# SilvioWeging/kASA

Hardware: AMD Instinct MI355X
Metric: reads/s in identify (10M x 150bp vs k=12 index) (higher is better)
Workload: dtype u64

## Files before the change

kasa_amd/csrc/kasa_hip.hip:

```cpp
#include <hip/hip_runtime.h>
#include <chrono>
#include <cstdlib>
#include <cstring>
#include <rocprim/device/device_radix_sort.hpp>
#include <rocprim/device/device_segmented_radix_sort.hpp>
#include <rocprim/iterator/transform_iterator.hpp>
#include <rocprim/device/device_scan.hpp>
#include <rocprim/functional.hpp>
#include <rocprim/iterator/counting_iterator.hpp>

#include <algorithm>
#include <cstdarg>
#include <cstdint>
#include <cstdio>
#include <cstring>
#include <map>
#include <mutex>
#include <new>
#include <string>
#include <thread>
#include <type_traits>
#include <vector>

#include <dlfcn.h>
// ... 4921 lines not shown
#pragma unroll
        for (int c = 0; c < HELD; ++c) if ((uint32_t)c * 64u < m) pass1((uint32_t)c * 64u, held[c]);
        for (uint32_t i0 = HELD * 64u; i0 < m; i0 += 64) {
            const uint32_t i = i0 + lane;
            pass1(i0, i < m ? st[s0 + i] : make_uint2(RK_FINAL, 0u));
        }
        LDS_WAVE_SYNC();
        uint32_t carry = 0;
        for (uint32_t w0 = 0; w0 < W; w0 += 64) {
            const uint32_t w = w0 + lane;
            const uint32_t pc = (w < W) ? (uint32_t)__popc(bm[w]) : 0u;
            uint32_t incl = pc;
            incl = wave_incl_sum(incl);
            if (w < W) pre[w] = carry + incl - pc;
            carry += lane_value<63>(incl);
        }
        const uint32_t nSlots = carry;
        LDS_WAVE_SYNC();
        auto pass2 = [&](uint32_t i0, uint2 e) {
            const uint32_t i = i0 + lane;
            bool pending = false;
            uint32_t slot = 0;
            float sc = 0.0f;
            if (i < m) {
                const uint32_t kind = e.x >> 30;
                if (kind != 2u) {
                    const uint32_t t = e.x & 0xFFFFFu;
                    slot = pre[t >> 5] + (uint32_t)__popc(bm[t >> 5] & ((1u << (t & 31u)) - 1u));
                    slotTax[slot] = t;
                    if (kind == 1u) val[slot] = __uint_as_float(e.y);
                    else { pending = true; if (kind == 0u) sc = event_score(evT, kHigh - (int)rk_level(e.x), e.y >> 16); }
                }
            }
            while (__ballot(pending) != 0ull) {
                if (pending) atomicMin(&claim[slot], (uint32_t)lane);
                LDS_WAVE_SYNC();
                if (pending && claim[slot] == (uint32_t)lane) {
                    float v = val[slot];
                    if ((e.x >> 30) == 3u) {
                        const int kF = (int)((e.x >> 20) & 31u), kL = (int)(e.y & 31u);
                        const int step = (e.x & RK_SEG_DESC) ? -1 : 1;
                        for (int k = step > 0 ? kF : kL, c = kL - kF; c >= 0; --c, k += step)
                            v = __fadd_rn(v, event_score(evT, k, seg_size(e.y, k == kF)));
                    } else
                        for (uint32_t j = 0; j < (e.y & 0xFFFFu); ++j) v = __fadd_rn(v, sc);
                    val[slot] = v;
                    claim[slot] = 0xFFFFFFFFu;
                    pending = false;
                }
                LDS_WAVE_SYNC();
            }
        };
#pragma unroll
        for (int c = 0; c < HELD; ++c) if ((uint32_t)c * 64u < m) pass2((uint32_t)c * 64u, held[c]);
        for (uint32_t i0 = HELD * 64u; i0 < m; i0 += 64) {
            const uint32_t i = i0 + lane;
            pass2(i0, i < m ? st[s0 + i] : make_uint2(0u, 0u));
        }
        LDS_WAVE_SYNC();
        for (uint32_t sl = lane; sl < nSlots; sl += 64) st[s0 + sl] = make_uint2(slotTax[sl], __float_as_uint(val[sl]));
        if (lane == 0) rowLen[r] = nSlots;
        LDS_WAVE_SYNC();
#pragma unroll
        for (int c = 0; c < HELD; ++c) held[c] = ahead[c];
    }
}

static constexpr int PR_THREADS = 256, PR_ITEMS = 8;
__global__ __launch_bounds__(PR_THREADS) void profile_reduce_kernel(const uint64_t *__restrict__ sorted, uint32_t nKeys, uint32_t nTaxa,
                                                                     uint64_t *__restrict__ cntUnique, uint64_t *__restrict__ hiTab,
                                                                     uint64_t *__restrict__ midTab, uint64_t *__restrict__ loTab, ProfLayout PL)
{
    __shared__ unsigned long long sSum[PR_THREADS / 64];
    __shared__ uint64_t sEdge[2];
    const uint64_t mask = (1ull << PL.bits()) - 1ull;
    auto add = [&](uint64_t key, uint64_t c) {
        const uint32_t tax = (uint32_t)(key & ((1ull << PL.tb) - 1ull));
        if (c == 0 || tax == (1u << PL.tb) - 1u) return;
        const uint32_t n = (uint32_t)((key >> PL.tb) & ((1ull << PL.nb) - 1ull));
        const uint32_t lv = (uint32_t)(key >> (PL.tb + PL.nb));
        const size_t cell = (size_t)lv * nTaxa + tax;
        if (n == 1) atomicAdd((unsigned long long *)&cntUnique[cell], (unsigned long long)c);
        fixed_add(hiTab, midTab, loTab, cell, c, n);
    };
    const uint32_t chunk = PR_THREADS * PR_ITEMS;
    for (uint64_t base = (uint64_t)blockIdx.x * chunk; base < nKeys; base += (uint64_t)gridDim.x * chunk) {
        const uint64_t i0 = base + threadIdx.x * PR_ITEMS;
        uint64_t v[PR_ITEMS];
        if (i0 + PR_ITEMS <= nKeys) {
#pragma unroll
            for (int j = 0; j < PR_ITEMS; j += 2) {
                const ulonglong2 w = *reinterpret_cast<const ulonglong2 *>(sorted + i0 + j);
                v[j] = w.x; v[j + 1] = w.y;
            }
        } else {
#pragma unroll
            for (int j = 0; j < PR_ITEMS; ++j) v[j] = (i0 + j < nKeys) ? sorted[i0 + j] : ~0ull;
        }
        if (threadIdx.x == 0) sEdge[0] = (v[0] >> 16) & mask;
        const uint32_t lastIdx = (base + chunk <= nKeys) ? chunk - 1 : (uint32_t)(nKeys - 1 - base);
        if (threadIdx.x == lastIdx / PR_ITEMS) sEdge[1] = (v[lastIdx % PR_ITEMS] >> 16) & mask;
        __syncthreads();
        const bool uniform = sEdge[0] == sEdge[1];
        if (uniform) {
            unsigned long long sum = 0;
#pragma unroll
            for (int j = 0; j < PR_ITEMS; ++j) if (i0 + j < nKeys) sum += v[j] & 0xFFFFull;
            for (int off = 32; off > 0; off >>= 1) sum += __shfl_down(sum, off);
            if ((threadIdx.x & 63) == 0) sSum[threadIdx.x >> 6] = sum;
            __syncthreads();
            if (threadIdx.x == 0) {
                unsigned long long total = 0;
                for (int w = 0; w < PR_THREADS / 64; ++w) total += sSum[w];
                add(sEdge[0], total);
            }
        } else {
            uint64_t cur = (v[0] >> 16) & mask, acc = 0;
#pragma unroll
            for (int j = 0; j < PR_ITEMS; ++j) {
                if (i0 + j >= nKeys) break;
                const uint64_t k = (v[j] >> 16) & mask;
                if (k != cur) { add(cur, acc); cur = k; acc = 0; }
                acc += v[j] & 0xFFFFull;
            }
            add(cur, acc);
        }
        __syncthreads();
    }
}

static constexpr int PT_THREADS = 1024, PT_LEFT = 2048;
struct ProfTableLayout { uint8_t nn[MAX_LEVELS]; uint16_t first[MAX_LEVELS + 1]; int lvLo, lvHi; };
static ProfTableLayout prof_table_layout(int nK, int lvLo, int lvHi, uint32_t nTaxa, uint64_t budgetCells)
{
    ProfTableLayout L;
    memset(&L, 0, sizeof(L));
    L.lvLo = lvLo; L.lvHi = lvHi;
    const uint64_t perTaxon = nTaxa ? budgetCells / nTaxa : 0;
    const int nW = lvHi - lvLo;
    if (nW <= 0 || perTaxon < (uint64_t)nW) { L.lvHi = lvLo; return L; }
    uint64_t left = perTaxon - (uint64_t)nW;
    for (int lv = lvLo; lv < lvHi; ++lv) L.nn[lv] = 1;
    auto grow = [&](int lv, uint64_t upTo) { while (lv >= lvLo && lv < lvHi && L.nn[lv] < upTo && left > 0) { ++L.nn[lv]; --left; } };
    for (int lv = lvLo; lv < lvHi; ++lv) grow(lv, 2);
    if (lvHi == nK) {
        grow(nK - 2, 4);
        grow(nK - 1, 24);
        grow(nK - 2, 8);
    }
    for (uint64_t upTo = 3; upTo <= 8; ++upTo) for (int lv = lvHi - 1; lv >= lvLo; --lv) grow(lv, upTo);
    for (int lv = 0; lv < MAX_LEVELS; ++lv) L.first[lv + 1] = (uint16_t)(L.first[lv] + L.nn[lv]);
    return L;
}
__global__ __launch_bounds__(PT_THREADS) void profile_table_kernel(const uint64_t *__restrict__ keys, uint32_t nKeys, uint32_t nTaxa, int nK, ProfTableLayout TL,
                                                                   uint64_t *__restrict__ cntUnique, uint64_t *__restrict__ hiTab,
                                                                   uint64_t *__restrict__ midTab, uint64_t *__restrict__ loTab, ProfLayout PL,
                                                                   uint64_t *__restrict__ leftOut, unsigned long long *__restrict__ leftCursor)
{
    extern __shared__ uint32_t tab[];
    __shared__ uint64_t sLeft[PT_LEFT];
    __shared__ uint32_t sLeftN;
    __shared__ unsigned long long sLeftBase;
    const uint32_t cells = (uint32_t)TL.first[MAX_LEVELS] * nTaxa;
    for (uint32_t i = threadIdx.x; i < cells; i += PT_THREADS) tab[i] = 0u;
    if (threadIdx.x == 0) sLeftN = 0;
    __syncthreads();
    const uint64_t mask = (1ull << PL.bits()) - 1ull;
    auto flush0 = [&]() {
        const uint32_t n = min(sLeftN, (uint32_t)PT_LEFT);
        if (threadIdx.x == 0) sLeftBase = atomicAdd(leftCursor, (unsigned long long)n);
        __syncthreads();
        for (uint32_t i = threadIdx.x; i < n; i += PT_THREADS) leftOut[sLeftBase + i] = sLeft[i];
        __syncthreads();
        if (threadIdx.x == 0) sLeftN = 0;
        __syncthreads();
    };
    constexpr int PT_KEYS = 8;
    const uint64_t step = (uint64_t)gridDim.x * PT_THREADS * PT_KEYS;
    const uint64_t rounds = ((uint64_t)nKeys + step - 1) / step;
    const uint32_t maxHits = (uint32_t)std::min<uint64_t>(65535ull, 0xFFFFFFFFull / std::max<uint64_t>(1, rounds * PT_THREADS * PT_KEYS));
    auto &flush = flush0;
    for (uint64_t rd = 0; rd < rounds; ++rd) {
        const uint64_t i0 = rd * step + (uint64_t)blockIdx.x * PT_THREADS * PT_KEYS + threadIdx.x;
        uint64_t kk[PT_KEYS];
#pragma unroll
        for (int q = 0; q < PT_KEYS; ++q) { const uint64_t i = i0 + (uint64_t)q * PT_THREADS; kk[q] = i < nKeys ? keys[i] : 0ull; }
#pragma unroll
        for (int q = 0; q < PT_KEYS; ++q) {
            const uint64_t key = kk[q];
            const uint64_t f = (key >> 16) & mask;
            const uint32_t hits = (uint32_t)(key & 0xFFFFull);
            const uint32_t tax = (uint32_t)(f & ((1ull << PL.tb) - 1ull));
            if (hits != 0u && tax != (1u << PL.tb) - 1u) {
                const uint32_t n = (uint32_t)((f >> PL.tb) & ((1ull << PL.nb) - 1ull));
                const uint32_t lv = (uint32_t)(f >> (PL.tb + PL.nb));
                if ((int)lv < TL.lvLo || (int)lv >= TL.lvHi) {}
                else if (n >= 1u && n <= (uint32_t)TL.nn[lv] && hits <= maxHits) atomicAdd(&tab[((uint32_t)TL.first[lv] + (n - 1u)) * nTaxa + tax], hits);
                else {
                    const uint32_t at = atomicAdd(&sLeftN, 1u);
                    if (at < (uint32_t)PT_LEFT) sLeft[at] = key;
                    else leftOut[atomicAdd(leftCursor, 1ull)] = key;
                }
            }
        }
        __syncthreads();
        if (sLeftN > (uint32_t)(PT_LEFT / 2)) flush();
    }
    flush();
    for (uint32_t i = threadIdx.x; i < cells; i += PT_THREADS) {
        const uint32_t c = tab[i];
        if (!c) continue;
        const uint32_t tax = i % nTaxa, row = i / nTaxa;
        uint32_t lv = 0;
        while (row >= (uint32_t)TL.first[lv + 1]) ++lv;
        const uint32_t n = row - (uint32_t)TL.first[lv] + 1u;
        const size_t cell = (size_t)lv * nTaxa + tax;
        if (n == 1u) atomicAdd((unsigned long long *)&cntUnique[cell], (unsigned long long)c);
        fixed_add(hiTab, midTab, loTab, cell, c, n);
    }
}

__global__ __launch_bounds__(256) void row_copy_kernel(const uint32_t *__restrict__ rowPos, const uint32_t *__restrict__ rowLen,
                                const uint64_t *__restrict__ rowOff, uint32_t nReads, const uint2 *__restrict__ st,
                                uint32_t *__restrict__ outTax, float *__restrict__ outScore)
{
    const int lane = threadIdx.x & 63, wv = threadIdx.x >> 6;
    const uint32_t waves = gridDim.x * 4u;
    for (uint32_t r = blockIdx.x * 4u + wv; r < nReads; r += waves) {
        const uint32_t s = rowPos[r];
        const uint32_t m = rowLen[r] & ~ROW_MERGE;
        const uint64_t o = rowOff[r];
        for (uint32_t i = lane; i < m; i += 64) { const uint2 e = st[s + i]; outTax[o + i] = e.x; outScore[o + i] = __uint_as_float(e.y); }
    }
}

__global__ void widen_kernel(const uint32_t *__restrict__ in, uint64_t *__restrict__ out, uint32_t n)
{
    const uint32_t i = blockIdx.x * blockDim.x + threadIdx.x;
    if (i < n) out[i] = in[i] & 0x7FFFFFFFu;
}

__global__ void invert_kernel(const uint32_t *__restrict__ plist, uint32_t n, uint32_t *__restrict__ slotOf)
{
    const uint32_t i = blockIdx.x * blockDim.x + threadIdx.x;
    if (i < n) slotOf[plist[i]] = i;
}

static int slots_from_reads(kasa_ctx *c)
{
    const uint64_t nQ = c->nQ;
    int rc;
    if ((rc = c->plist.reserve(nQ * 4 + 64)) || (rc = c->slotBuf.reserve(nQ * 4 + 64)) || (rc = c->qReadA.reserve(nQ * 4 + 64))) return rc;
    hipEvent_t a, b;
    if ((rc = timer_begin(c, c->timers[KASA_STAGE_REGROUP], &a, &b))) return rc;
    if (nQ) {
        unsigned bits = 1;
        while ((1ull << bits) < (uint64_t)std::max<int64_t>(c->nReads, 1)) ++bits;
        rocprim::counting_iterator<uint32_t> iota(0);
        size_t tmpBytes = 0;
        HIPCHK(rocprim::radix_sort_pairs(nullptr, tmpBytes, c->qRead, c->qReadA.as<uint32_t>(), iota, c->plist.as<uint32_t>(),
                                         (size_t)nQ, 0u, bits, c->stream));
        if ((rc = c->sortTmp.reserve(tmpBytes))) return rc;
        HIPCHK(rocprim::radix_sort_pairs(c->sortTmp.p, tmpBytes, c->qRead, c->qReadA.as<uint32_t>(), iota, c->plist.as<uint32_t>(),
                                         (size_t)nQ, 0u, bits, c->stream));
        invert_kernel<<<blocks_for(nQ, 256), 256, 0, c->stream>>>(c->plist.as<uint32_t>(), (uint32_t)nQ, c->slotBuf.as<uint32_t>());
        HIPCHK(hipGetLastError());
    }
    if ((rc = timer_end(c, c->timers[KASA_STAGE_REGROUP], a, b))) return rc;
    c->slotOf = c->slotBuf.as<uint32_t>();
    return KASA_OK;
}

template <int RW>
static int launch_group(kasa_ctx *c, const uint32_t *slotOf, uint32_t nTiles, uint32_t cap, uint32_t keyCap, int cov, unsigned long long *cursor, bool coop,
                        const uint32_t *tileList = nullptr, uint32_t nListed = 0)
{
    const uint64_t nQ = c->nQ;
    uint32_t *needCoop = reinterpret_cast<uint32_t *>(cursor + 3);
    const uint32_t grid = tileList ? nListed : nTiles;
#define KASA_GROUP_ARGS(KEY, META) c->keys<KEY>(), c->depth.as<uint8_t>(), c->rep.as<uint32_t>(), slotOf, (uint32_t)nQ, \
        c->tileNext.as<uint32_t>(), nTiles, c->ix->meta.as<META>(), c->ix->tax.as<uint32_t>(), (uint32_t)c->ix->n, \
        c->kHigh, c->kLow, c->recOut ? c->recOut : c->rec.as<uint32_t>(), c->pool.as<uint32_t>(), cap, cursor, cov, c->cntTotal.as<uint64_t>(), c->ix->nTaxa, \
        c->profKeys.as<uint64_t>(), keyCap, cursor + 2, prof_layout(c->ix->nTaxa, c->nK), c->cntAllHi.as<uint64_t>(), c->cntAllMid.as<uint64_t>(), c->cntAllLo.as<uint64_t>(), needCoop, tileList, c->recOut ? (uint32_t)RW : c->recCW
    if (c->ix->wide && RW == 16 && c->nK == 19)
        group_kernel<RW, key128, RW == 16 ? 19 : 0><<<grid, GTHREADS, 0, c->stream>>>(KASA_GROUP_ARGS(key128, uint16_t));
    else if (c->ix->wide)
        group_kernel<RW, key128, 0><<<grid, GTHREADS, 0, c->stream>>>(KASA_GROUP_ARGS(key128, uint16_t));
    else if (RW == 8 && c->nK == 6) {
        if (coop) group_kernel<RW, uint64_t, RW == 8 ? 6 : 0, RW == 8><<<grid, GTHREADS, 0, c->stream>>>(KASA_GROUP_ARGS(uint64_t, uint8_t));
        else group_kernel<RW, uint64_t, RW == 8 ? 6 : 0><<<grid, GTHREADS, 0, c->stream>>>(KASA_GROUP_ARGS(uint64_t, uint8_t));
    } else if (coop && RW == 8)
        group_kernel<RW, uint64_t, 0, RW == 8><<<grid, GTHREADS, 0, c->stream>>>(KASA_GROUP_ARGS(uint64_t, uint8_t));
    else
        group_kernel<RW, uint64_t, 0><<<grid, GTHREADS, 0, c->stream>>>(KASA_GROUP_ARGS(uint64_t, uint8_t));
#undef KASA_GROUP_ARGS
    HIPCHK(hipGetLastError());
    return KASA_OK;
}

static int launch_group2(kasa_ctx *c, const uint32_t *slotOf, uint32_t nTiles, uint32_t cap, uint32_t keyCap, int cov, unsigned long long *cursor, uint32_t *slowCount,
                         const uint32_t *tileIn = nullptr, uint32_t nIn = 0, uint32_t *slowListOut = nullptr)
{
    const uint64_t nQ = c->nQ;
#define KASA_GROUP2_ARGS(KEY, META) c->keys<KEY>(), c->depth.as<uint8_t>(), c->rep.as<uint32_t>(), slotOf, (uint32_t)nQ, \
        c->tileNext.as<uint32_t>(), nTiles, c->ix->meta.as<META>(), c->ix->tax.as<uint32_t>(), (uint32_t)c->ix->n, \
        c->kHigh, c->kLow, c->recOut ? c->recOut : c->rec.as<uint32_t>(), c->pool.as<uint32_t>(), cap, cursor, cov, c->ix->nTaxa, \
        c->profKeys.as<uint64_t>(), keyCap, cursor + 2, prof_layout(c->ix->nTaxa, c->nK), c->cntAllHi.as<uint64_t>(), c->cntAllMid.as<uint64_t>(), c->cntAllLo.as<uint64_t>(), \
        slowCount, slowListOut ? slowListOut : c->tileList.as<uint32_t>(), c->recOut ? 8u : c->recCW, tileIn
    static const size_t pad = getenv("KASA_G2_PADLDS") ? (size_t)atoi(getenv("KASA_G2_PADLDS")) : 0;
    const uint32_t grid = tileIn ? nIn : nTiles;
    if (tileIn) group2_kernel<uint64_t, 6, 0, 4><<<grid, GTHREADS, 0, c->stream>>>(KASA_GROUP2_ARGS(uint64_t, uint8_t));
    else
    if (c->ix->wide) group2_kernel<key128, 0><<<grid, GTHREADS, pad, c->stream>>>(KASA_GROUP2_ARGS(key128, uint16_t));
    else if (c->nK == 6) {
#ifdef KASA_G2_VARIANTS
        static const int var = getenv("KASA_G2_VAR") ? atoi(getenv("KASA_G2_VAR")) : 0;
        if (var == 1) group2_kernel<uint64_t, 6, 1><<<grid, GTHREADS, pad, c->stream>>>(KASA_GROUP2_ARGS(uint64_t, uint8_t));
        else if (var == 2) group2_kernel<uint64_t, 6, 2><<<grid, GTHREADS, pad, c->stream>>>(KASA_GROUP2_ARGS(uint64_t, uint8_t));
        else if (var == 3) group2_kernel<uint64_t, 6, 3><<<grid, GTHREADS, pad, c->stream>>>(KASA_GROUP2_ARGS(uint64_t, uint8_t));
        else if (var == 4) group2_kernel<uint64_t, 6, 4><<<grid, GTHREADS, pad, c->stream>>>(KASA_GROUP2_ARGS(uint64_t, uint8_t));
        else
#endif
        group2_kernel<uint64_t, 6><<<grid, GTHREADS, pad, c->stream>>>(KASA_GROUP2_ARGS(uint64_t, uint8_t));
    }
    else group2_kernel<uint64_t, 0><<<grid, GTHREADS, pad, c->stream>>>(KASA_GROUP2_ARGS(uint64_t, uint8_t));
#undef KASA_GROUP2_ARGS
    HIPCHK(hipGetLastError());
    return KASA_OK;
}


__global__ __launch_bounds__(PT_THREADS) void profile_group_table_kernel(const uint64_t *__restrict__ keys, uint32_t nKeys, uint32_t nTaxa, int nK, ProfTableLayout TL,
                                                                         uint64_t *__restrict__ cntUnique, uint64_t *__restrict__ hiTab,
                                                                         uint64_t *__restrict__ midTab, uint64_t *__restrict__ loTab, ProfLayout PL,
                                                                         uint64_t *__restrict__ leftOut, unsigned long long *__restrict__ leftCursor, unsigned long long leftCap,
                                                                         int rangeCells)
{
    extern __shared__ uint32_t tab[];
    const uint32_t cells = (uint32_t)TL.first[MAX_LEVELS] * nTaxa;
    uint32_t *tabR = tab + cells;
    const uint32_t rangeN = rangeCells ? (uint32_t)nK * nTaxa : 0u;
    __shared__ uint32_t sWave[PT_THREADS / 64];
    __shared__ unsigned long long sBase;
    for (uint32_t i = threadIdx.x; i < cells + rangeN; i += PT_THREADS) tab[i] = 0u;
    __syncthreads();
    const int lane = (int)(threadIdx.x & 63u), wv = (int)(threadIdx.x >> 6);
    auto direct = [&](uint32_t lv, uint32_t n, uint32_t tax, uint32_t hits) {
        const size_t cell = (size_t)lv * nTaxa + tax;
        if (n == 1u) atomicAdd((unsigned long long *)&cntUnique[cell], (unsigned long long)hits);
        fixed_add(hiTab, midTab, loTab, cell, hits, n);
    };
    constexpr int PT_KEYS = 8;
    const uint64_t step = (uint64_t)gridDim.x * PT_THREADS * PT_KEYS;
    const uint64_t rounds = ((uint64_t)nKeys + step - 1) / step;
    const uint32_t maxHits = (uint32_t)std::min<uint64_t>(65535ull, 0xFFFFFFFFull / std::max<uint64_t>(1, rounds * PT_THREADS * PT_KEYS));
    for (uint64_t rd = 0; rd < rounds; ++rd) {
        const uint64_t i0 = rd * step + (uint64_t)blockIdx.x * PT_THREADS * PT_KEYS + threadIdx.x;
        uint64_t kk[PT_KEYS];
#pragma unroll
        for (int q = 0; q < PT_KEYS; ++q) { const uint64_t i = i0 + (uint64_t)q * PT_THREADS; kk[q] = i < nKeys ? keys[i] : 0ull; }
        auto levelsOf = [&](uint64_t key, auto cell, auto left) {
            const uint32_t hits = (uint32_t)(key & 0xFFFFull);
            if (hits == 0u) return;
            const uint32_t tax = (uint32_t)(key >> 16) & SEG_TAX_MASK, n = (uint32_t)(key >> 38) & 0x1FFFu;
            const uint32_t lvLo = (uint32_t)(key >> 51) & 31u, lvHi = lvLo + ((uint32_t)(key >> 56) & 31u);
            if (rangeN && n == 1u && lvHi + 1u == (uint32_t)nK && hits <= maxHits) { cell(&tabR[lvLo * nTaxa + tax], hits); return; }
            for (uint32_t lv = lvLo; lv <= lvHi; ++lv) {
                if ((int)lv >= TL.lvLo && (int)lv < TL.lvHi && n >= 1u && n <= (uint32_t)TL.nn[lv] && hits <= maxHits) cell(&tab[((uint32_t)TL.first[lv] + (n - 1u)) * nTaxa + tax], hits);
                else left(lv, n, tax, hits);
            }
        };
        uint32_t nLeft = 0;
        unsigned long long which = 0;
#pragma unroll
        for (int q = 0; q < PT_KEYS; ++q)
            levelsOf(kk[q], [&](uint32_t *c, uint32_t hits) { atomicAdd(c, hits); }, [&](uint32_t lv, uint32_t, uint32_t, uint32_t) { ++nLeft; which |= 1ull << (8 * q + (int)(lv & 7u)); });
        const uint32_t incl = wave_incl_sum(nLeft);
        if (lane == 63) sWave[wv] = incl;
        __syncthreads();
        uint32_t before = 0, total = 0;
        for (int w = 0; w < PT_THREADS / 64; ++w) { const uint32_t o = sWave[w]; if (w < wv) before += o; total += o; }
        if (total == 0u) { __syncthreads(); continue; }
        if (threadIdx.x == 0) sBase = atomicAdd(leftCursor, (unsigned long long)total);
        __syncthreads();
        unsigned long long at = sBase + before + incl - nLeft;
        if (nLeft && nK <= 8) {
#pragma unroll
            for (int q = 0; q < PT_KEYS; ++q) {
                uint32_t m = (uint32_t)(which >> (8 * q)) & 255u;
                const uint64_t key = kk[q];
                const uint32_t hits = (uint32_t)(key & 0xFFFFull), tax = (uint32_t)(key >> 16) & SEG_TAX_MASK, n = (uint32_t)(key >> 38) & 0x1FFFu;
                while (m) {
                    const uint32_t lv = (uint32_t)__ffs((int)m) - 1u;
                    m &= m - 1u;
                    if (at < leftCap) leftOut[at] = profile_key_of(lv, n, tax, hits, PL); else direct(lv, n, tax, hits);
                    ++at;
                }
            }
        } else if (nLeft) {
#pragma unroll
            for (int q = 0; q < PT_KEYS; ++q)
                levelsOf(kk[q], [&](uint32_t *, uint32_t) {}, [&](uint32_t lv, uint32_t n, uint32_t tax, uint32_t hits) {
                    if (at < leftCap) leftOut[at] = profile_key_of(lv, n, tax, hits, PL); else direct(lv, n, tax, hits);
                    ++at;
                });
        }
        __syncthreads();
    }
    __syncthreads();
    if (rangeN)
        for (uint32_t tax = threadIdx.x; tax < nTaxa; tax += PT_THREADS) {
            unsigned long long acc = 0;
            for (int lv = 0; lv < nK; ++lv) {
                acc += tabR[(uint32_t)lv * nTaxa + tax];
                if (!acc) continue;
                const size_t cell = (size_t)lv * nTaxa + tax;
                atomicAdd((unsigned long long *)&cntUnique[cell], acc);
                atomicAdd((unsigned long long *)&hiTab[cell], acc);
            }
        }
    for (uint32_t i = threadIdx.x; i < cells; i += PT_THREADS) {
        const uint32_t c = tab[i];
        if (!c) continue;
        const uint32_t tax = i % nTaxa, row = i / nTaxa;
        uint32_t lv = 0;
        while (row >= (uint32_t)TL.first[lv + 1]) ++lv;
        const uint32_t n = row - (uint32_t)TL.first[lv] + 1u;
        const size_t cell = (size_t)lv * nTaxa + tax;
        if (n == 1u) atomicAdd((unsigned long long *)&cntUnique[cell], (unsigned long long)c);
        fixed_add(hiTab, midTab, loTab, cell, c, n);
    }
}

static constexpr int PA_THREADS = 1024, PA_NMAX = 8192;
__global__ void profile_rtab_kernel(uint64_t *__restrict__ rTab)
{
    const uint32_t n = blockIdx.x * blockDim.x + threadIdx.x;
    if (n >= (uint32_t)PA_NMAX) return;
    uint64_t R = n ? 0xFFFFFFFFFFFFFFFFull / n : 0ull;
    if (n && (n & (n - 1)) == 0) R += 1;
    rTab[n] = R;
}
__global__ __launch_bounds__(PA_THREADS) void profile_group_accum_kernel(const uint64_t *__restrict__ keys, uint32_t nKeys, uint32_t nTaxa, int winLo, int winHi,
                                                                         const uint64_t *__restrict__ rTab, uint64_t *__restrict__ cntUnique, uint64_t *__restrict__ hiTab,
                                                                         uint64_t *__restrict__ midTab, uint64_t *__restrict__ loTab)
{
    extern __shared__ unsigned long long shAcc[];
    const uint32_t cells = (uint32_t)(winHi - winLo) * nTaxa;
    unsigned long long *sA = shAcc, *sB = shAcc + cells, *sCU = shAcc + 2 * (size_t)cells;
    auto flush = [&]() {
        __syncthreads();
        for (uint32_t i = threadIdx.x; i < cells; i += PA_THREADS) {
            const unsigned long long a = sA[i], b = sB[i], cu = sCU[i];
            if ((a | b | cu) == 0ull) continue;
            const size_t cell = (size_t)winLo * nTaxa + i;
            if (a) atomicAdd((unsigned long long *)&loTab[cell], a);
            if (b) atomicAdd((unsigned long long *)&midTab[cell], b);
            if (cu & 0xFFFFFFFFull) atomicAdd((unsigned long long *)&hiTab[cell], cu & 0xFFFFFFFFull);
            if (cu >> 32) atomicAdd((unsigned long long *)&cntUnique[cell], cu >> 32);
            sA[i] = 0ull; sB[i] = 0ull; sCU[i] = 0ull;
        }
        __syncthreads();
    };
    for (uint32_t i = threadIdx.x; i < 3u * cells; i += PA_THREADS) shAcc[i] = 0ull;
    __syncthreads();
    const uint64_t step = (uint64_t)gridDim.x * PA_THREADS;
    uint32_t sinceFlush = 0;
    for (uint64_t i0 = (uint64_t)blockIdx.x * PA_THREADS; i0 < nKeys; i0 += step) {
        const uint64_t i = i0 + threadIdx.x;
        const uint64_t key = i < nKeys ? keys[i] : 0ull;
        const uint32_t hits = (uint32_t)(key & 0xFFFFull);
        if (hits) {
            const uint32_t tax = (uint32_t)(key >> 16) & SEG_TAX_MASK, n = (uint32_t)(key >> 38) & 0x1FFFu;
            int lo = (int)((key >> 51) & 31u), hi = lo + (int)((key >> 56) & 31u);
            lo = lo < winLo ? winLo : lo; hi = hi >= winHi ? winHi - 1 : hi;
            if (lo <= hi && hits >= 256u) {
                for (int lv = lo; lv <= hi; ++lv) {
                    const size_t cell = (size_t)lv * nTaxa + tax;
                    if (n == 1u) atomicAdd((unsigned long long *)&cntUnique[cell], (unsigned long long)hits);
                    fixed_add(hiTab, midTab, loTab, cell, hits, n);
                }
            } else if (lo <= hi) {
                unsigned long long a = 0, b = 0, cu;
                if (n == 1u) cu = (unsigned long long)hits | ((unsigned long long)hits << 32);
                else {
                    const uint64_t R = rTab[n];
                    const uint64_t lo64 = (uint64_t)hits * R;
                    a = lo64 & 0xFFFFFFFFull; b = lo64 >> 32; cu = __umul64hi((uint64_t)hits, R);
                }
                for (int lv = lo; lv <= hi; ++lv) {
                    const uint32_t cell = (uint32_t)(lv - winLo) * nTaxa + tax;
                    if (a) atomicAdd(&sA[cell], a);
                    if (b) atomicAdd(&sB[cell], b);
                    if (cu) atomicAdd(&sCU[cell], cu);
                }
            }
        }
        sinceFlush += PA_THREADS;
        if (sinceFlush >= (1u << 22)) { flush(); sinceFlush = 0; }
    }
    flush();
}

static int profile_from_keys(kasa_ctx *c, uint64_t nKeys, bool grouped)
{
    if (nKeys == 0) return KASA_OK;
    const uint32_t nTaxa = c->ix->nTaxa;
    const int nK = c->nK;
    int rc;
    hipStream_t ps = c->stream;
    static const char *timing = getenv("KASA_PROF_TIMING");
    auto now = [&]() { if (timing) (void)hipStreamSynchronize(ps); return std::chrono::steady_clock::now(); };
    const auto t0 = now();
    const ProfLayout PL = prof_layout(nTaxa, nK);
    const bool accum = grouped && !(c->debugFlags & 67108864) && (c->groupCoop || c->profLeftHint > nKeys / 4 || (c->debugFlags & 268435456));
    if (accum) {
        const uint64_t budget = 152u * 1024u;
        const int perPass = (int)std::min<uint64_t>((uint64_t)nK, budget / ((uint64_t)nTaxa * 24u));
        if (perPass >= 1 && (nK + perPass - 1) / perPass <= 3) {
            if (!c->rTab.p) {
                if ((rc = c->rTab.reserve((size_t)PA_NMAX * 8))) return rc;
                profile_rtab_kernel<<<PA_NMAX / 256, 256, 0, ps>>>(c->rTab.as<uint64_t>());
                HIPCHK(hipGetLastError());
            }
            int nCu = 0;
            HIPCHK(hipDeviceGetAttribute(&nCu, hipDeviceAttributeMultiprocessorCount, c->device));
            for (int lo = 0; lo < nK; lo += perPass) {
                const int hi = std::min(nK, lo + perPass);
                const size_t shBytes = (size_t)(hi - lo) * nTaxa * 24;
                HIPCHK(hipFuncSetAttribute((const void *)profile_group_accum_kernel, hipFuncAttributeMaxDynamicSharedMemorySize, (int)shBytes));
                profile_group_accum_kernel<<<std::max(1, nCu), PA_THREADS, shBytes, ps>>>(c->profKeys.as<uint64_t>(), (uint32_t)nKeys, nTaxa, lo, hi,
                    c->rTab.as<uint64_t>(), c->cntUnique.as<uint64_t>(), c->cntAllHi.as<uint64_t>(), c->cntAllMid.as<uint64_t>(), c->cntAllLo.as<uint64_t>());
                HIPCHK(hipGetLastError());
            }
            if (timing) { const auto t1 = now(); fprintf(stderr, "kasa: profile keys %llu: exact LDS accumulation, %d level(s) per pass, %.1f ms\n", (unsigned long long)nKeys, perPass, std::chrono::duration<double>(t1 - t0).count() * 1e3); }
            return KASA_OK;
        }
    }
    uint64_t leftCap = grouped ? std::max<uint64_t>(std::max<uint64_t>(nKeys / 4, 1u << 20), c->profLeftHint) : std::max<uint64_t>(nKeys, 1u << 20);
    leftCap = std::min<uint64_t>(leftCap, 0xFFFFFFF0ull);
    if ((rc = c->profSorted.reserve((size_t)leftCap * 8 + 64))) return rc;
    if (grouped && (rc = c->profSorted2.reserve((size_t)leftCap * 8 + 64))) return rc;
    uint64_t budgetCells = (160u * 1024u - PT_LEFT * 8u - 1024u) / 4u;
    const bool rangeCells = grouped && (uint64_t)nK * nTaxa <= budgetCells / 3;
    if (rangeCells) budgetCells -= (uint64_t)nK * nTaxa;
    std::vector<ProfTableLayout> passes;
    if (nK <= 8 || grouped) passes.push_back(prof_table_layout(nK, 0, nK, nTaxa, budgetCells));
    else {
        passes.push_back(prof_table_layout(nK, nK - 4, nK, nTaxa, budgetCells));
        for (int hi = nK - 4; hi > 0; hi -= 8) passes.push_back(prof_table_layout(nK, std::max(0, hi - 8), hi, nTaxa, budgetCells));
    }
    bool tables = !(c->debugFlags & 16) || grouped;
    for (const auto &TL : passes) if (TL.lvHi <= TL.lvLo && !grouped) tables = false;
    uint64_t *sortIn = c->profKeys.as<uint64_t>(), *sortOut = c->profSorted.as<uint64_t>();
    uint64_t nSort = nKeys;
    if (tables) {
        int nCu = 0;
        HIPCHK(hipDeviceGetAttribute(&nCu, hipDeviceAttributeMultiprocessorCount, c->device));
        unsigned long long *leftCursor = c->misc.as<unsigned long long>() + 19;
        unsigned long long left = 0;
        HIPCHK(hipMemsetAsync(leftCursor, 0, 8, ps));
        for (const auto &TL : passes) {
            const size_t shBytes = ((size_t)TL.first[MAX_LEVELS] * nTaxa + (rangeCells ? (size_t)nK * nTaxa : 0)) * 4;
            HIPCHK(hipFuncSetAttribute((const void *)profile_table_kernel, hipFuncAttributeMaxDynamicSharedMemorySize, (int)shBytes));
            if (grouped) {
                HIPCHK(hipFuncSetAttribute((const void *)profile_group_table_kernel, hipFuncAttributeMaxDynamicSharedMemorySize, (int)shBytes));
                profile_group_table_kernel<<<std::max(1, nCu), PT_THREADS, shBytes, ps>>>(c->profKeys.as<uint64_t>(), (uint32_t)nKeys, nTaxa, nK, TL,
                    c->cntUnique.as<uint64_t>(), c->cntAllHi.as<uint64_t>(), c->cntAllMid.as<uint64_t>(), c->cntAllLo.as<uint64_t>(), PL,
                    c->profSorted.as<uint64_t>(), leftCursor, (unsigned long long)leftCap, rangeCells ? 1 : 0);
            } else
            profile_table_kernel<<<std::max(1, nCu), PT_THREADS, shBytes, ps>>>(c->profKeys.as<uint64_t>(), (uint32_t)nKeys, nTaxa, nK, TL,
                c->cntUnique.as<uint64_t>(), c->cntAllHi.as<uint64_t>(), c->cntAllMid.as<uint64_t>(), c->cntAllLo.as<uint64_t>(), PL,
                c->profSorted.as<uint64_t>(), leftCursor);
            HIPCHK(hipGetLastError());
        }
        HIPCHK(hipMemcpyAsync(&left, leftCursor, 8, hipMemcpyDeviceToHost, ps));
        HIPCHK(hipStreamSynchronize(ps));
        nSort = std::min<uint64_t>(left, leftCap); sortIn = c->profSorted.as<uint64_t>();
        sortOut = grouped ? c->profSorted2.as<uint64_t>() : c->profKeys.as<uint64_t>();
        if (grouped && left > leftCap) c->profLeftHint = left + left / 4;
    }
    const auto t1 = now();
    if (nSort > 0) {
        const int sortBits = (int)((PL.bits() + 7u) / 8u) * 8;
        if ((rc = c->sortTmp.reserve(kasa_radix::scratch_bytes<uint64_t>(nSort)))) return rc;
        uint64_t *kRes = nullptr;
        HIPCHK(kasa_radix::sort_pairs<uint64_t>(sortIn, nullptr, sortOut, nullptr, (uint32_t)nSort, 16, sortBits, c->sortTmp.p, ps, &kRes, nullptr));
        profile_reduce_kernel<<<std::min<unsigned>(blocks_for(nSort, PR_THREADS * PR_ITEMS), 256u * 16u), PR_THREADS, 0, ps>>>(
            kRes, (uint32_t)nSort, nTaxa,
            c->cntUnique.as<uint64_t>(), c->cntAllHi.as<uint64_t>(), c->cntAllMid.as<uint64_t>(), c->cntAllLo.as<uint64_t>(), PL);
        HIPCHK(hipGetLastError());
    }
    if (timing) {
        const auto t2 = now();
        fprintf(stderr, "kasa: profile keys %llu: tables %.1f ms, %llu left over (list %llu), sort + reduce %.1f ms\n", (unsigned long long)nKeys,
                std::chrono::duration<double>(t1 - t0).count() * 1e3, (unsigned long long)nSort, (unsigned long long)leftCap, std::chrono::duration<double>(t2 - t1).count() * 1e3);
    }
    return KASA_OK;
}

static int group_stage(kasa_ctx *c, int coverage, bool exportSorted, uint32_t *recordsOut = nullptr)
{
    if (c->state < 3) return fail(KASA_E_STATE, "kasa_batch_group: batch not sorted");
    HIPCHK(hipSetDevice(c->ix->device));
    const uint64_t nQ = c->nQ;
    const int RW = c->recWords();
    int rc;
    c->haveScores = false; c->nnz = 0; c->grouped = false; c->poolUsed = 1; c->recSorted = exportSorted; c->recOut = exportSorted ? recordsOut : nullptr;
    if (nQ == 0) { c->grouped = true; return KASA_OK; }
    if (!exportSorted && !c->slotOf && (rc = slots_from_reads(c))) return rc;
    const uint32_t nTiles = (uint32_t)((nQ + TILE - 1) / TILE);
    c->recCW = (uint32_t)RW;
    static const bool cellsEnv = getenv("KASA_WIDE_CELLS") && atoi(getenv("KASA_WIDE_CELLS")) != 0;
    if (RW == 8 && !exportSorted && !c->noWideCells && !c->groupCoop && !coverage && (cellsEnv || (c->debugFlags & 134217728)) && !(c->debugFlags & (16777216 | 2048 | 131072 | 262144))) {
        if (c->rec.cap < nQ * (size_t)64 + 64) {
            size_t freeB = 0, totalB = 0;
            HIPCHK(hipMemGetInfo(&freeB, &totalB));
            if (freeB + c->rec.cap < nQ * (size_t)64 + 64 + ((size_t)24 << 30)) c->noWideCells = true;
        }
        if (!c->noWideCells) c->recCW = 16u;
    }
    if (!c->recOut && (rc = (RW == 8 && c->recCW == 8u) ? reserve_placed(c->rec, nQ * (size_t)32 + 64, c->stream, &c->recPlacement)
                                                          : c->rec.reserve(nQ * (size_t)c->recCW * 4 + 64))) return rc;
    unsigned long long *cursor = c->misc.as<unsigned long long>() + 16;
    hipEvent_t a, b;
    if (c->poolCap == 0) c->poolCap = std::max<uint64_t>(1u << 16, nQ);
    if (c->keyCap == 0) c->keyCap = RW == 8 ? std::max<uint64_t>(1u << 20, nQ / 2 + nQ / 4) : 64;
    uint64_t nKeys = 0;
    for (int attempt = 0;; ++attempt) {
        if (c->keyCap >= 0xFFFFFFF0ull) return fail(KASA_E_LIMIT, "the profile of this batch needs %llu keys (limit 2^32); split the batch", (unsigned long long)c->keyCap);
        if ((rc = c->pool.reserve(c->poolCap * 4)) || (rc = c->profKeys.reserve(c->keyCap * 8 + 64))) return rc;
        const unsigned long long one = 1, zero = 0;
        HIPCHK(hipMemcpyAsync(cursor, &one, 8, hipMemcpyHostToDevice, c->stream));
        HIPCHK(hipMemcpyAsync(cursor + 2, &zero, 8, hipMemcpyHostToDevice, c->stream));
        if ((rc = timer_begin(c, c->timers[KASA_STAGE_GROUP], &a, &b))) return rc;
        const uint32_t cap = (uint32_t)std::min<uint64_t>(c->poolCap, 0xFFFFFFF0ull);
        static const int g2tap = getenv("KASA_G2_TAP") ? atoi(getenv("KASA_G2_TAP")) : 0;
        static const int longSteps = getenv("KASA_LONG_STEPS") ? (atoi(getenv("KASA_LONG_STEPS")) & 127) : 0;
        const int cov = (g2tap & (32 | 64 | 128 | 256)) | ((longSteps ? longSteps : (c->groupCoop ? (int)LONG_STEPS_CROWDED : 0)) << 9) | ((coverage && attempt == 0) ? 1 : 0) | ((c->debugFlags & 2048) ? 2 : 0) | ((c->debugFlags & 4096) ? 4 : 0) | ((c->debugFlags & 32768) ? 8 : 0) | ((c->debugFlags & 65536) ? 16 : 0);
        const uint32_t *slotOf = exportSorted ? nullptr : c->slotOf;
        hipEvent_t ka, kb;
        if ((rc = timer_begin(c, c->kernels[KASA_KERNEL_GROUP], &ka, &kb))) return rc;
        HIPCHK(hipMemcpyAsync(cursor + 3, &zero, 8, hipMemcpyHostToDevice, c->stream));
        if (c->debugFlags & 262144) c->groupCoop = true;
        const bool coop = c->groupCoop && !(c->debugFlags & 131072);
        const bool g2 = RW == 8 && !coop && !(cov & 1) && !(c->debugFlags & (16777216 | 2048 | 131072));
        unsigned long long used[4] = {0, 0, 0, 0};
        if (g2) {
            if ((rc = c->tileList.reserve((size_t)nTiles * 8 + 256))) return rc;
            if ((rc = launch_group2(c, slotOf, nTiles, cap, (uint32_t)c->keyCap, cov, cursor, reinterpret_cast<uint32_t *>(cursor + 3) + 1))) return rc;
            HIPCHK(hipMemcpyAsync(used, cursor, 32, hipMemcpyDeviceToHost, c->stream));
            HIPCHK(hipStreamSynchronize(c->stream));
            const uint32_t nListed = (uint32_t)(used[3] >> 32);
            c->lastSlowTiles = nListed; c->lastSlowTiles2 = nListed;
            if (nListed && getenv("KASA_DEBUG_WHY")) {
                std::vector<uint32_t> h(nListed);
                HIPCHK(hipMemcpy(h.data(), c->tileList.p, (size_t)nListed * 4, hipMemcpyDeviceToHost));
                uint32_t why[8] = {0, 0, 0, 0, 0, 0, 0, 0};
                for (uint32_t x : h) why[(x >> 28) & 7u]++;
                fprintf(stderr, "[kasa] group2 left %u of %u tiles: long list %u, span %u, both %u, parked only %u, parked + long %u, parked + span %u, all %u\n",
                        nListed, nTiles, why[1], why[2], why[3], why[4], why[5], why[6], why[7]);
            }
            const uint32_t *coopList = c->tileList.as<uint32_t>();
            uint32_t nCoop = nListed;
            static const bool g2Always = getenv("KASA_G2_ALWAYS") && atoi(getenv("KASA_G2_ALWAYS")) != 0;
            if (nListed && c->nK == 6 && !c->ix->wide && !(cov & (32 | 64 | 128 | 256)) && ((uint64_t)nListed * 4 <= nTiles || g2Always) && !getenv("KASA_NO_SECOND_CHANCE")) {
                uint32_t *count2 = c->misc.as<uint32_t>() + 78, *list2 = c->tileList.as<uint32_t>() + nTiles + 16;
                HIPCHK(hipMemsetAsync(count2, 0, 4, c->stream));
                if ((rc = launch_group2(c, slotOf, nTiles, cap, (uint32_t)c->keyCap, cov, cursor, count2, c->tileList.as<uint32_t>(), nListed, list2))) return rc;
                uint32_t n2 = 0;
                HIPCHK(hipMemcpyAsync(&n2, count2, 4, hipMemcpyDeviceToHost, c->stream));
                HIPCHK(hipStreamSynchronize(c->stream));
                coopList = list2; nCoop = n2;
                c->lastSlowTiles2 = n2;
                if (getenv("KASA_DEBUG_WHY")) fprintf(stderr, "[kasa] group2's second launch left %u of %u listed tiles to the cooperative kernel\n", n2, nListed);
            }
            if (nCoop && (rc = launch_group<8>(c, slotOf, nTiles, cap, (uint32_t)c->keyCap, cov, cursor, true, coopList, nCoop))) return rc;
            if ((uint64_t)nListed * 4 > nTiles && !(getenv("KASA_G2_ALWAYS") && atoi(getenv("KASA_G2_ALWAYS")) != 0)) c->groupCoop = true;
        } else {
            c->lastSlowTiles = 0; c->lastSlowTiles2 = 0;
            if ((rc = (RW == 8 ? launch_group<8>(c, slotOf, nTiles, cap, (uint32_t)c->keyCap, cov, cursor, coop) : launch_group<16>(c, slotOf, nTiles, cap, (uint32_t)c->keyCap, cov, cursor, false)))) return rc;
        }
        if ((rc = timer_end(c, c->kernels[KASA_KERNEL_GROUP], ka, kb))) return rc;
        if ((rc = timer_end(c, c->timers[KASA_STAGE_GROUP], a, b))) return rc;
        HIPCHK(hipMemcpyAsync(used, cursor, 32, hipMemcpyDeviceToHost, c->stream));
        HIPCHK(hipStreamSynchronize(c->stream));
        if (g2 && (used[3] & 1ull)) return fail(KASA_E_LIMIT, "a query meets 255 or more taxa of a 128-bit index through narrow records; use the index's own k range");
        if (RW == 8 && !g2 && !coop && !(c->debugFlags & 131072) && ((used[3] & 1ull) || used[0] > 6ull * nQ)) {
            c->groupCoop = true;
            if (used[3] & 1ull) { if (used[0] > c->poolCap) c->poolCap = used[0] + used[0] / 8 + 1024; continue; }
        }
        if (used[0] <= c->poolCap && used[2] <= c->keyCap) { c->poolUsed = (uint32_t)used[0]; nKeys = used[2]; break; }
        if (used[0] >= 0xFFFFFFF0ull) return fail(KASA_E_LIMIT, "the taxon lists of this batch need %llu pool entries (limit 2^32); split the batch", used[0]);
        if (used[0] > c->poolCap) c->poolCap = used[0] + used[0] / 8 + 1024;
        if (used[2] > c->keyCap) c->keyCap = used[2] + used[2] / 8 + 1024;
        if (attempt > 3) return fail(KASA_E_LIMIT, "taxon-list pool did not converge");
    }
    if ((rc = timer_begin(c, c->timers[KASA_STAGE_GROUP], &a, &b))) return rc;
    {
        hipEvent_t ka, kb;
        if ((rc = timer_begin(c, c->kernels[KASA_KERNEL_PROFILE_TABLES], &ka, &kb))) return rc;
        if (RW == 8 && (rc = profile_from_keys(c, nKeys, true))) return rc;
        if ((rc = timer_end(c, c->kernels[KASA_KERNEL_PROFILE_TABLES], ka, kb))) return rc;
    }
    if ((rc = timer_end(c, c->timers[KASA_STAGE_GROUP], a, b))) return rc;
    c->lastKeys = nKeys;
    c->grouped = true;
    return KASA_OK;
}

template <int RW>
static int launch_flush(kasa_ctx *c, const uint32_t *list, uint32_t nList, const uint64_t *flushOff, uint32_t *out)
{
    const uint32_t nTiles = (uint32_t)((c->nQ + TILE - 1) / TILE);
    const unsigned blocks = std::min<uint32_t>(nList, 256u * 32u);
    if (c->ix->wide)
// ... 2406 lines not shown
```

Baseline: 57.99 million.

## Pack profile table layout into 64-bit words and restructure grouped accumulation loop

Replaces the per-level layout arrays passed to the profile table kernels with two packed 64-bit words (byte per level), so layout lookups become shifts on registers instead of indexed parameter loads. The grouped kernel now loads keys as 128-bit vectors, prefetches the next round's keys before processing, and computes level masks per key, then walks levels outer and keys inner to issue shared atomics. It drops the generic fallback path for more than eight levels and instead rejects such configurations with an error. This trades generality for fewer dynamic indexing and branching costs in the profiling stage.

```diff
diff --git a/kasa_amd/csrc/kasa_hip.hip b/kasa_amd/csrc/kasa_hip.hip
--- a/kasa_amd/csrc/kasa_hip.hip
+++ b/kasa_amd/csrc/kasa_hip.hip
@@ -5097,7 +5097,25 @@
     for (int lv = 0; lv < MAX_LEVELS; ++lv) L.first[lv + 1] = (uint16_t)(L.first[lv] + L.nn[lv]);
     return L;
 }
-__global__ __launch_bounds__(PT_THREADS) void profile_table_kernel(const uint64_t *__restrict__ keys, uint32_t nKeys, uint32_t nTaxa, int nK, ProfTableLayout TL,
+struct ProfTablePacked {
+    uint64_t nnPk, firstPk;
+    int lvLo, lvHi;
+    uint32_t rows;
+    __device__ __forceinline__ uint32_t nn(uint32_t j) const { return (uint32_t)(nnPk >> (8u * j)) & 255u; }
+    __device__ __forceinline__ uint32_t first(uint32_t j) const { return (uint32_t)(firstPk >> (8u * j)) & 255u; }
+    __device__ __forceinline__ uint32_t level_of_row(uint32_t row) const { uint32_t j = 0; while (j < 7u && row >= first(j) + nn(j)) ++j; return j; }
+};
+static bool prof_table_pack(const ProfTableLayout &L, ProfTablePacked &P)
+{
+    P.nnPk = 0; P.firstPk = 0; P.lvLo = L.lvLo; P.lvHi = L.lvHi; P.rows = L.first[MAX_LEVELS];
+    if (L.lvHi - L.lvLo > 8 || L.first[MAX_LEVELS] > 255u) return false;
+    for (int j = 0; j < 8 && L.lvLo + j < MAX_LEVELS; ++j) {
+        P.nnPk |= (uint64_t)L.nn[L.lvLo + j] << (8 * j);
+        P.firstPk |= (uint64_t)L.first[L.lvLo + j] << (8 * j);
+    }
+    return true;
+}
+__global__ __launch_bounds__(PT_THREADS) void profile_table_kernel(const uint64_t *__restrict__ keys, uint32_t nKeys, uint32_t nTaxa, int nK, ProfTablePacked TL,
                                                                    uint64_t *__restrict__ cntUnique, uint64_t *__restrict__ hiTab,
                                                                    uint64_t *__restrict__ midTab, uint64_t *__restrict__ loTab, ProfLayout PL,
                                                                    uint64_t *__restrict__ leftOut, unsigned long long *__restrict__ leftCursor)
@@ -5106,7 +5124,8 @@
     __shared__ uint64_t sLeft[PT_LEFT];
     __shared__ uint32_t sLeftN;
     __shared__ unsigned long long sLeftBase;
-    const uint32_t cells = (uint32_t)TL.first[MAX_LEVELS] * nTaxa;
+    const uint32_t cells = TL.rows * nTaxa;
+    const uint32_t nW = (uint32_t)(TL.lvHi - TL.lvLo);
     for (uint32_t i = threadIdx.x; i < cells; i += PT_THREADS) tab[i] = 0u;
     if (threadIdx.x == 0) sLeftN = 0;
     __syncthreads();
@@ -5139,8 +5158,9 @@
             if (hits != 0u && tax != (1u << PL.tb) - 1u) {
                 const uint32_t n = (uint32_t)((f >> PL.tb) & ((1ull << PL.nb) - 1ull));
                 const uint32_t lv = (uint32_t)(f >> (PL.tb + PL.nb));
-                if ((int)lv < TL.lvLo || (int)lv >= TL.lvHi) {}
-                else if (n >= 1u && n <= (uint32_t)TL.nn[lv] && hits <= maxHits) atomicAdd(&tab[((uint32_t)TL.first[lv] + (n - 1u)) * nTaxa + tax], hits);
+                const uint32_t j = lv - (uint32_t)TL.lvLo;
+                if (j >= nW) {}
+                else if (n >= 1u && n <= TL.nn(j) && hits <= maxHits) atomicAdd(&tab[(TL.first(j) + (n - 1u)) * nTaxa + tax], hits);
                 else {
                     const uint32_t at = atomicAdd(&sLeftN, 1u);
                     if (at < (uint32_t)PT_LEFT) sLeft[at] = key;
@@ -5156,9 +5176,8 @@
         const uint32_t c = tab[i];
         if (!c) continue;
         const uint32_t tax = i % nTaxa, row = i / nTaxa;
-        uint32_t lv = 0;
-        while (row >= (uint32_t)TL.first[lv + 1]) ++lv;
-        const uint32_t n = row - (uint32_t)TL.first[lv] + 1u;
+        const uint32_t j = TL.level_of_row(row), lv = (uint32_t)TL.lvLo + j;
+        const uint32_t n = row - TL.first(j) + 1u;
         const size_t cell = (size_t)lv * nTaxa + tax;
         if (n == 1u) atomicAdd((unsigned long long *)&cntUnique[cell], (unsigned long long)c);
         fixed_add(hiTab, midTab, loTab, cell, c, n);
@@ -5275,14 +5294,14 @@
 }
 
 
-__global__ __launch_bounds__(PT_THREADS) void profile_group_table_kernel(const uint64_t *__restrict__ keys, uint32_t nKeys, uint32_t nTaxa, int nK, ProfTableLayout TL,
+__global__ __launch_bounds__(PT_THREADS) void profile_group_table_kernel(const uint64_t *__restrict__ keys, uint32_t nKeys, uint32_t nTaxa, int nK, ProfTablePacked TL,
                                                                          uint64_t *__restrict__ cntUnique, uint64_t *__restrict__ hiTab,
                                                                          uint64_t *__restrict__ midTab, uint64_t *__restrict__ loTab, ProfLayout PL,
                                                                          uint64_t *__restrict__ leftOut, unsigned long long *__restrict__ leftCursor, unsigned long long leftCap,
                                                                          int rangeCells)
 {
     extern __shared__ uint32_t tab[];
-    const uint32_t cells = (uint32_t)TL.first[MAX_LEVELS] * nTaxa;
+    const uint32_t cells = TL.rows * nTaxa;
     uint32_t *tabR = tab + cells;
     const uint32_t rangeN = rangeCells ? (uint32_t)nK * nTaxa : 0u;
     __shared__ uint32_t sWave[PT_THREADS / 64];
@@ -5299,27 +5318,51 @@
     const uint64_t step = (uint64_t)gridDim.x * PT_THREADS * PT_KEYS;
     const uint64_t rounds = ((uint64_t)nKeys + step - 1) / step;
     const uint32_t maxHits = (uint32_t)std::min<uint64_t>(65535ull, 0xFFFFFFFFull / std::max<uint64_t>(1, rounds * PT_THREADS * PT_KEYS));
+    auto firstOf = [&](uint64_t rd, int q) { return rd * step + (uint64_t)blockIdx.x * PT_THREADS * PT_KEYS + (uint64_t)q * PT_THREADS + 2u * threadIdx.x; };
+    auto load = [&](uint64_t (&k)[PT_KEYS], uint64_t rd) {
+#pragma unroll
+        for (int q = 0; q < PT_KEYS; q += 2) {
+            const uint64_t i = firstOf(rd, q);
+            const ulonglong2 w = *reinterpret_cast<const ulonglong2 *>(keys + (i < nKeys ? i : 0ull));
+            k[q] = w.x; k[q + 1] = w.y;
+        }
+    };
+    uint64_t nx[PT_KEYS];
+    load(nx, 0);
     for (uint64_t rd = 0; rd < rounds; ++rd) {
-        const uint64_t i0 = rd * step + (uint64_t)blockIdx.x * PT_THREADS * PT_KEYS + threadIdx.x;
         uint64_t kk[PT_KEYS];
 #pragma unroll
-        for (int q = 0; q < PT_KEYS; ++q) { const uint64_t i = i0 + (uint64_t)q * PT_THREADS; kk[q] = i < nKeys ? keys[i] : 0ull; }
-        auto levelsOf = [&](uint64_t key, auto cell, auto left) {
+        for (int q = 0; q < PT_KEYS; q += 2) {
+            const uint64_t i = firstOf(rd, q);
+            kk[q] = i < nKeys ? nx[q] : 0ull; kk[q + 1] = i + 1 < nKeys ? nx[q + 1] : 0ull;
+        }
+        load(nx, rd + 1);
+        uint32_t hitsOf[PT_KEYS], nm1[PT_KEYS], cellOf[PT_KEYS];
+        unsigned long long which = 0;
+#pragma unroll
+        for (int q = 0; q < PT_KEYS; ++q) {
+            const uint64_t key = kk[q];
             const uint32_t hits = (uint32_t)(key & 0xFFFFull);
-            if (hits == 0u) return;
             const uint32_t tax = (uint32_t)(key >> 16) & SEG_TAX_MASK, n = (uint32_t)(key >> 38) & 0x1FFFu;
             const uint32_t lvLo = (uint32_t)(key >> 51) & 31u, lvHi = lvLo + ((uint32_t)(key >> 56) & 31u);
-            if (rangeN && n == 1u && lvHi + 1u == (uint32_t)nK && hits <= maxHits) { cell(&tabR[lvLo * nTaxa + tax], hits); return; }
-            for (uint32_t lv = lvLo; lv <= lvHi; ++lv) {
-                if ((int)lv >= TL.lvLo && (int)lv < TL.lvHi && n >= 1u && n <= (uint32_t)TL.nn[lv] && hits <= maxHits) cell(&tab[((uint32_t)TL.first[lv] + (n - 1u)) * nTaxa + tax], hits);
-                else left(lv, n, tax, hits);
-            }
-        };
-        uint32_t nLeft = 0;
-        unsigned long long which = 0;
-#pragma unroll
-        for (int q = 0; q < PT_KEYS; ++q)
-            levelsOf(kk[q], [&](uint32_t *c, uint32_t hits) { atomicAdd(c, hits); }, [&](uint32_t lv, uint32_t, uint32_t, uint32_t) { ++nLeft; which |= 1ull << (8 * q + (int)(lv & 7u)); });
+            hitsOf[q] = hits;
+            nm1[q] = hits <= maxHits ? n - 1u : ~0u;
+            cellOf[q] = (n - 1u) * nTaxa + tax;
+            if (hits == 0u) continue;
+            if (rangeN && n == 1u && lvHi + 1u == (uint32_t)nK && hits <= maxHits) { atomicAdd(&tabR[lvLo * nTaxa + tax], hits); continue; }
+            which |= (unsigned long long)(((2u << (lvHi & 7u)) - (1u << (lvLo & 7u))) & 255u) << (8 * q);
+        }
+#pragma unroll
+        for (int lv = 0; lv < 8; ++lv) {
+            if (lv >= nK) break;
+            const uint32_t nnL = TL.nn((uint32_t)lv), rowL = TL.first((uint32_t)lv) * nTaxa;
+#pragma unroll
+            for (int q = 0; q < PT_KEYS; ++q) {
+                const unsigned long long bit = 1ull << (8 * q + lv);
+                if ((which & bit) && nm1[q] < nnL) { atomicAdd(&tab[rowL + cellOf[q]], hitsOf[q]); which &= ~bit; }
+            }
+        }
+        const uint32_t nLeft = (uint32_t)__popcll(which);
         const uint32_t incl = wave_incl_sum(nLeft);
         if (lane == 63) sWave[wv] = incl;
         __syncthreads();
@@ -5329,7 +5372,7 @@
         if (threadIdx.x == 0) sBase = atomicAdd(leftCursor, (unsigned long long)total);
         __syncthreads();
         unsigned long long at = sBase + before + incl - nLeft;
-        if (nLeft && nK <= 8) {
+        if (nLeft) {
 #pragma unroll
             for (int q = 0; q < PT_KEYS; ++q) {
                 uint32_t m = (uint32_t)(which >> (8 * q)) & 255u;
@@ -5342,13 +5385,6 @@
                     ++at;
                 }
             }
-        } else if (nLeft) {
-#pragma unroll
-            for (int q = 0; q < PT_KEYS; ++q)
-                levelsOf(kk[q], [&](uint32_t *, uint32_t) {}, [&](uint32_t lv, uint32_t n, uint32_t tax, uint32_t hits) {
-                    if (at < leftCap) leftOut[at] = profile_key_of(lv, n, tax, hits, PL); else direct(lv, n, tax, hits);
-                    ++at;
-                });
         }
         __syncthreads();
     }
@@ -5368,9 +5404,8 @@
         const uint32_t c = tab[i];
         if (!c) continue;
         const uint32_t tax = i % nTaxa, row = i / nTaxa;
-        uint32_t lv = 0;
-        while (row >= (uint32_t)TL.first[lv + 1]) ++lv;
-        const uint32_t n = row - (uint32_t)TL.first[lv] + 1u;
+        const uint32_t lv = TL.level_of_row(row);
+        const uint32_t n = row - TL.first(lv) + 1u;
         const size_t cell = (size_t)lv * nTaxa + tax;
         if (n == 1u) atomicAdd((unsigned long long *)&cntUnique[cell], (unsigned long long)c);
         fixed_add(hiTab, midTab, loTab, cell, c, n);
@@ -5505,8 +5540,10 @@
         unsigned long long *leftCursor = c->misc.as<unsigned long long>() + 19;
         unsigned long long left = 0;
         HIPCHK(hipMemsetAsync(leftCursor, 0, 8, ps));
-        for (const auto &TL : passes) {
-            const size_t shBytes = ((size_t)TL.first[MAX_LEVELS] * nTaxa + (rangeCells ? (size_t)nK * nTaxa : 0)) * 4;
+        for (const auto &L : passes) {
+            ProfTablePacked TL;
+            if (!prof_table_pack(L, TL) || (grouped && nK > 8)) return fail(KASA_E_LIMIT, "profile tables: a window of more than eight levels");
+            const size_t shBytes = ((size_t)TL.rows * nTaxa + (rangeCells ? (size_t)nK * nTaxa : 0)) * 4;
             HIPCHK(hipFuncSetAttribute((const void *)profile_table_kernel, hipFuncAttributeMaxDynamicSharedMemorySize, (int)shBytes));
             if (grouped) {
                 HIPCHK(hipFuncSetAttribute((const void *)profile_group_table_kernel, hipFuncAttributeMaxDynamicSharedMemorySize, (int)shBytes));
```

After: 59.39 million, median of 6. +2.4%, better.
